# BloodAxe/pytorch-toolbelt

Hardware: AMD Instinct MI355X
Metric: megapixels/sec tiled+d4-TTA merge on 5000x5000 (higher is better)
Workload: dtype f32

## Files before the change

### pytorch_toolbelt_amd/csrc/ptb_channels_last.hip

```cpp
#include "ptb_dispatch.h"
#include "ptb_view_device.h"

namespace ptb {

namespace {

constexpr int CL_THREADS = 256;
constexpr int CL_NC = 4;

template <int IN> struct LdOf { static constexpr int value = IN == PTB_F32 ? 0 : (IN == PTB_F16 ? 2 : 3); };

template <int IN, bool VEC>
__device__ __forceinline__ float4 cl_load(const float* base, long long off, int nc) {
    if constexpr (VEC) {
        return ld4<LdOf<IN>::value>(base, off);
    } else {
        float4 v = make_float4(1.f, 1.f, 1.f, 1.f);
        v.x = widen<IN>(base, off);
        if (nc > 1) v.y = widen<IN>(base, off + 1);
        if (nc > 2) v.z = widen<IN>(base, off + 2);
        if (nc > 3) v.w = widen<IN>(base, off + 3);
        return v;
    }
}

template <int OPK, int IN, bool VEC>
__device__ __forceinline__ float4 cl_reduce_px(const float* __restrict__ base, long long off0, long long view_stride, int nv, int codes, int H, int W,
                                               int C, int i, int j, int c0, int nc, int op, float divisor) {
    float4 v[MAX_VIEWS];
#pragma unroll
    for (int k = 0; k < MAX_VIEWS; ++k) {
        v[k] = make_float4(1.f, 1.f, 1.f, 1.f);
        if (k < nv) {
            const int code = (codes >> (3 * k)) & 7;
            int rr = (code & 1) ? j : i, cc = (code & 1) ? i : j;
            const int rows = (code & 1) ? W : H, cols = (code & 1) ? H : W;
            if (code & 2) rr = rows - 1 - rr;
            if (code & 4) cc = cols - 1 - cc;
            v[k] = cl_load<IN, VEC>(base, off0 + (long long)k * view_stride + ((long long)rr * cols + cc) * C + c0, nc);
        }
    }
    float4 s = make_float4(red_pre<OPK>(v[0].x, op), red_pre<OPK>(v[0].y, op), red_pre<OPK>(v[0].z, op), red_pre<OPK>(v[0].w, op));
#pragma unroll
    for (int k = 1; k < MAX_VIEWS; ++k) {
        if (k < nv) {
            s.x = __fadd_rn(s.x, red_pre<OPK>(v[k].x, op));
            s.y = __fadd_rn(s.y, red_pre<OPK>(v[k].y, op));
            s.z = __fadd_rn(s.z, red_pre<OPK>(v[k].z, op));
            s.w = __fadd_rn(s.w, red_pre<OPK>(v[k].w, op));
        }
    }
    return make_float4(red_post<OPK>(s.x, op, divisor), red_post<OPK>(s.y, op, divisor), red_post<OPK>(s.z, op, divisor),
                       red_post<OPK>(s.w, op, divisor));
}

template <int OPK, int IN, bool VEC>
__device__ __forceinline__ void cl_blend(const ViewArgs& a, const float* __restrict__ base, long long off0, long long view_stride, int li, int lj, int c0,
                                         int nc, float w, float4& acc) {
    const float4 val = round_src4<LdOf<IN>::value>(
        cl_reduce_px<OPK, IN, VEC>(base, off0, view_stride, a.nviews, a.codes, a.H, a.W, a.C, li, lj, c0, nc, a.op, a.divisor), a.round_src);
    acc.x = __fadd_rn(acc.x, __fmul_rn(val.x, w));
    acc.y = __fadd_rn(acc.y, __fmul_rn(val.y, w));
    acc.z = __fadd_rn(acc.z, __fmul_rn(val.z, w));
    acc.w = __fadd_rn(acc.w, __fmul_rn(val.w, w));
}

__device__ __forceinline__ float4 cl_load_planes(const float* p, long long chan_stride, int nc) {
    float4 v = make_float4(0.f, 0.f, 0.f, 0.f);
    v.x = p[0];
    if (nc > 1) v.y = p[chan_stride];
    if (nc > 2) v.z = p[2 * chan_stride];
    if (nc > 3) v.w = p[3 * chan_stride];
    return v;
}
__device__ __forceinline__ void cl_store_planes(float* p, long long chan_stride, int nc, const float4 v) {
    p[0] = v.x;
    if (nc > 1) p[chan_stride] = v.y;
    if (nc > 2) p[2 * chan_stride] = v.z;
    if (nc > 3) p[3 * chan_stride] = v.w;
}
__device__ __forceinline__ float4 cl_div(const float4 s, float n) {
    return make_float4(__fdiv_rn(s.x, n), __fdiv_rn(s.y, n), __fdiv_rn(s.z, n), __fdiv_rn(s.w, n));
}

}

template <int OPK, int IN, bool VEC>
__global__ __launch_bounds__(CL_THREADS) void cl_reduce_kernel(const ViewArgs a, int chrows) {
    const int cpt = a.chunks_x * a.chunks_y;
    const int chunk = blockIdx.x % cpt, t = blockIdx.x / cpt;
    const int cx0 = (chunk % a.chunks_x) * CW, cy0 = (chunk / a.chunks_x) * chrows;
    const int cw = min(CW, a.W - cx0), ch = min(chrows, a.H - cy0);
    const int tx = threadIdx.x & 15, ty = threadIdx.x >> 4;
    const long long off0 = (long long)t * a.src_tile_stride;
    for (int r = ty; r < ch; r += 16) {
        for (int x = tx; x < cw; x += 16) {
            const int i = cy0 + r, j = cx0 + x;
            float* o = a.dst + (long long)t * a.dst_tile_stride + (long long)i * a.dst_row_stride + j;
            for (int c0 = 0; c0 < a.C; c0 += CL_NC) {
                const int nc = min(CL_NC, a.C - c0);
                const float4 val = cl_reduce_px<OPK, IN, VEC>(a.src, off0, a.src_view_stride, a.nviews, a.codes, a.H, a.W, a.C, i, j, c0, nc, a.op, a.divisor);
                cl_store_planes(o + (long long)c0 * a.dst_chan_stride, a.dst_chan_stride, nc, val);
            }
        }
    }
}

template <int OPK, int IN, bool VEC>
__global__ __launch_bounds__(CL_THREADS) void cl_accum_kernel(const ViewArgs a, const CellArgs g, int chrows) {
    const int chunk = blockIdx.x;
    int ci = 0;
    while (ci < a.ncells - 1 && chunk >= g.cells[ci].chunk_end) ++ci;
    const Cell& cell = g.cells[ci];
    const int first = ci ? g.cells[ci - 1].chunk_end : 0;
    const int ncx = (cell.w + CW - 1) / CW;
    const int lc = chunk - first;
    const int cx0 = (lc % ncx) * CW, cy0 = (lc / ncx) * chrows;
    const int cw = min(CW, cell.w - cx0), ch = min(chrows, cell.h - cy0);
    const int ax = cell.ox + cx0, ay = cell.oy + cy0;
    const int nt = cell.ntiles, fresh = cell.fresh, fin = cell.final_;
    const int tx = threadIdx.x & 15, ty = threadIdx.x >> 4;
    for (int r = ty; r < ch; r += 16) {
        for (int x = tx; x < cw; x += 16) {
            const long long pix = (long long)(ay + r) * a.dst_row_stride + ax + x;
            float wv[MAX_COVER];
#pragma unroll
            for (int e = 0; e < MAX_COVER; ++e) {
                wv[e] = 0.f;
                if (e < nt) {
                    const int gt = cell.tile[e];
                    wv[e] = a.weight[(long long)(ay + r - g.tile_y[gt]) * a.W + ax + x - g.tile_x[gt]];
                }
            }
            const float nfull = fin ? a.norm_full[pix] : 1.f;
            if (a.norm != nullptr && !fin) {
                float nacc = fresh ? 0.f : a.norm[pix];
#pragma unroll
                for (int e = 0; e < MAX_COVER; ++e)
                    if (e < nt) nacc = __fadd_rn(nacc, wv[e]);
                a.norm[pix] = nacc;
            }
            for (int c0 = 0; c0 < a.C; c0 += CL_NC) {
                const int nc = min(CL_NC, a.C - c0);
                float* ip = a.dst + (long long)c0 * a.dst_chan_stride + pix;
                float4 acc = fresh ? make_float4(0.f, 0.f, 0.f, 0.f) : cl_load_planes(ip, a.dst_chan_stride, nc);
#pragma unroll
                for (int e = 0; e < MAX_COVER; ++e) {
                    if (e < nt) {
                        const int gt = cell.tile[e];
                        cl_blend<OPK, IN, VEC>(a, a.src, (long long)g.tile_id[gt] * a.src_tile_stride, a.src_view_stride, ay + r - g.tile_y[gt],
                                               ax + x - g.tile_x[gt], c0, nc, wv[e], acc);
                    }
                }
                if (fin) {
                    cl_store_planes(a.merged + (long long)c0 * a.dst_chan_stride + pix, a.dst_chan_stride, nc, cl_div(acc, nfull));
                    if (a.keep_acc) cl_store_planes(ip, a.dst_chan_stride, nc, acc);
                } else {
                    cl_store_planes(ip, a.dst_chan_stride, nc, acc);
                }
            }
        }
    }
}

template <int OPK, int IN, bool VEC>
__global__ __launch_bounds__(CL_THREADS) void cl_band_kernel(const ViewArgs a, const BandArgs g) {
    constexpr int CH = 32;
    const int chunk = blockIdx.x;
    int ci = 0;
    while (ci < a.ncells - 1 && chunk >= g.cells[ci].chunk_end) ++ci;
    const BandCell& cell = g.cells[ci];
    const int first = ci ? g.cells[ci - 1].chunk_end : 0;
    const int ncx = (cell.w + CW - 1) / CW;
    const int lc = chunk - first;
    const int cx0 = (lc % ncx) * CW, cy0 = (lc / ncx) * CH;
    const int cw = min(CW, cell.w - cx0), ch = min(CH, cell.h - cy0);
    const int ax = cell.ox + cx0, ay = cell.oy + cy0;
    const int nt = cell.ntiles;
    const int tx = threadIdx.x & 15, ty = threadIdx.x >> 4;
    for (int r = ty; r < ch; r += 16) {
        for (int x = tx; x < cw; x += 16) {
            const long long pix = (long long)(ay + r) * a.dst_row_stride + ax + x;
            float wv[MAX_COVER];
#pragma unroll
            for (int e = 0; e < MAX_COVER; ++e) {
                wv[e] = 0.f;
                if (e < nt) {
                    const int gt = cell.tile[e];
                    wv[e] = a.weight[(long long)(ay + r - g.tile_y[gt]) * a.W + ax + x - g.tile_x[gt]];
                }
            }
            const float nfull = a.norm_full[pix];
            for (int c0 = 0; c0 < a.C; c0 += CL_NC) {
                const int nc = min(CL_NC, a.C - c0);
                float4 acc = make_float4(0.f, 0.f, 0.f, 0.f);
#pragma unroll
                for (int e = 0; e < MAX_COVER; ++e) {
                    if (e < nt) {
                        const int gt = cell.tile[e];
                        cl_blend<OPK, IN, VEC>(a, static_cast<const float*>(g.tile_src[gt]), 0, g.tile_vs[gt], ay + r - g.tile_y[gt], ax + x - g.tile_x[gt], c0,
                                               nc, wv[e], acc);
                    }
                }
                cl_store_planes(a.merged + (long long)c0 * a.dst_chan_stride + pix, a.dst_chan_stride, nc, cl_div(acc, nfull));
            }
        }
    }
}

template <int OPK, int IN, bool VEC>
__global__ __launch_bounds__(CL_THREADS) void cl_plan_kernel(const ViewArgs a, const BandItem* __restrict__ items, const GroupTiles t) {
    const BandItem* __restrict__ it = items + blockIdx.x;
    const int cwch = it->cwch, partial = it->partial, nt = it->ntiles;
    const int cw = cwch & 0xffff, ch = cwch >> 16;
    const int ax = it->ax, ay = it->ay;
    const int tx = threadIdx.x & 15, ty = threadIdx.x >> 4;
    for (int r = ty; r < ch; r += 16) {
        for (int x = tx; x < cw; x += 16) {
            const long long pix = (long long)(ay + r) * a.dst_row_stride + ax + x;
            float wv[MAX_COVER];
#pragma unroll
            for (int e = 0; e < MAX_COVER; ++e) {
                wv[e] = 0.f;
                if (e < nt) {
                    const unsigned long long cv = it->cover[e];
                    const int lx = (int)((cv >> 16) & 0xffff), ly = (int)((cv >> 32) & 0xffff);
                    wv[e] = a.weight[(long long)(ly + r) * a.W + lx + x];
                }
            }
            float nsum = (a.norm_map && !partial) ? a.norm_full[pix] : 0.f;
#pragma unroll
            for (int e = 0; e < MAX_COVER; ++e)
                if (e < nt && !a.norm_map) nsum = __fadd_rn(nsum, wv[e]);
            for (int c0 = 0; c0 < a.C; c0 += CL_NC) {
                const int nc = min(CL_NC, a.C - c0);
                float4 acc = make_float4(0.f, 0.f, 0.f, 0.f);
#pragma unroll
                for (int e = 0; e < MAX_COVER; ++e) {
                    if (e < nt) {
                        const unsigned long long cv = it->cover[e];
                        const int slot = (int)(cv & 0xffff), lx = (int)((cv >> 16) & 0xffff), ly = (int)((cv >> 32) & 0xffff);
                        cl_blend<OPK, IN, VEC>(a, static_cast<const float*>(t.src[slot]), 0, t.vs[slot], ly + r, lx + x, c0, nc, wv[e], acc);
                    }
                }
                cl_store_planes(a.merged + (long long)c0 * a.dst_chan_stride + pix, a.dst_chan_stride, nc, partial ? acc : cl_div(acc, nsum));
            }
        }
    }
}

template <class F>
static void with_cl_instance(const ViewArgs& a, bool vec, F&& f) {
    with_reduction(a.op, [&](auto opk) { with_src_dtype(a.in_dtype, [&](auto ld) { with_bool(vec, [&](auto v) {
        f(opk, int_c<ld_dtype<ld()>()>{}, v); }); }); });
}

static bool cl_vec_ok(const ViewArgs& a, const void* p, long long stride0, long long stride1) {
    const uintptr_t mask = a.in_dtype == PTB_F32 ? 15u : 7u;
    return a.C % 4 == 0 && (reinterpret_cast<uintptr_t>(p) & mask) == 0 && stride0 % 4 == 0 && stride1 % 4 == 0;
}

void cl_launch_reduce(const ViewArgs& a, int ntiles_out, int ch, hipStream_t s) {
    const dim3 grid((unsigned)ntiles_out * a.chunks_x * a.chunks_y);
    const bool vec = cl_vec_ok(a, a.src, a.src_tile_stride, a.src_view_stride);
    with_cl_instance(a, vec, [&](auto opk, auto in, auto v) {
        hipLaunchKernelGGL((cl_reduce_kernel<opk(), in(), v()>), grid, dim3(CL_THREADS), 0, s, a, ch); });
}

void cl_launch_accum(const ViewArgs& a, const CellArgs& g, int ch, hipStream_t s) {
    const dim3 grid((unsigned)a.total_chunks);
    const bool vec = cl_vec_ok(a, a.src, a.src_tile_stride, a.src_view_stride);
    with_cl_instance(a, vec, [&](auto opk, auto in, auto v) {
        hipLaunchKernelGGL((cl_accum_kernel<opk(), in(), v()>), grid, dim3(CL_THREADS), 0, s, a, g, ch); });
}

void cl_launch_band(const ViewArgs& a, const BandArgs& g, int chunks, hipStream_t s) {
    const dim3 grid((unsigned)chunks);
    bool vec = true;
    for (int ci = 0; ci < a.ncells; ++ci)
        for (int e = 0; e < g.cells[ci].ntiles; ++e) vec = vec && cl_vec_ok(a, g.tile_src[g.cells[ci].tile[e]], g.tile_vs[g.cells[ci].tile[e]], 0);
    with_cl_instance(a, vec, [&](auto opk, auto in, auto v) {
        hipLaunchKernelGGL((cl_band_kernel<opk(), in(), v()>), grid, dim3(CL_THREADS), 0, s, a, g); });
}

void cl_launch_plan(const ViewArgs& a, const BandItem* items, const GroupTiles& t, int n_items, hipStream_t s) {
    const dim3 grid((unsigned)n_items);
    bool vec = true;
    for (int k = 0; k < PLAN_TILES; ++k)
        if (t.src[k]) vec = vec && cl_vec_ok(a, t.src[k], t.vs[k], 0);
    with_cl_instance(a, vec, [&](auto opk, auto in, auto v) {
        hipLaunchKernelGGL((cl_plan_kernel<opk(), in(), v()>), grid, dim3(CL_THREADS), 0, s, a, items, t); });
}

}
```

### pytorch_toolbelt_amd/csrc/ptb_common.h

```cpp
#pragma once
#include <hip/hip_runtime.h>
#include <stdint.h>

#include <type_traits>

#include "../../include/ptb_hip.h"

namespace ptb {

void set_hip_error(hipError_t e);
void set_error_text(const char* text);

inline int check_launch() {
    hipError_t e = hipGetLastError();
    if (e != hipSuccess) {
        set_hip_error(e);
        return PTB_ELAUNCH;
    }
    return PTB_OK;
}

#ifndef PTB_NT_OUT
#define PTB_NT_OUT 1
#endif
__device__ __forceinline__ void out_store4(float* p, const float4 v) {
#if PTB_NT_OUT
    typedef float ptb_v4f __attribute__((ext_vector_type(4)));
    __builtin_nontemporal_store(ptb_v4f{v.x, v.y, v.z, v.w}, reinterpret_cast<ptb_v4f*>(p));
#else
    *reinterpret_cast<float4*>(p) = v;
#endif
}

__device__ __forceinline__ int wave_id() { return __builtin_amdgcn_readfirstlane((int)(threadIdx.x >> 6)); }

inline bool aligned16(const void* p) { return (reinterpret_cast<uintptr_t>(p) & 15u) == 0; }
inline long long up16(long long v) { return (v + 15) & ~15LL; }

inline bool bad_elem_bytes(int eb) { return eb != 1 && eb != 2 && eb != 4 && eb != 8; }
template <int EB>
using label_t = std::conditional_t<EB == 1, unsigned char, std::conditional_t<EB == 2, short, std::conditional_t<EB == 4, int, long long>>>;
inline bool holds(int elem_bytes, long long v) {
    switch (elem_bytes) {
        case 1: return v >= 0 && v <= 255;
        case 2: return v >= -32768 && v <= 32767;
        case 4: return v >= -2147483648LL && v <= 2147483647LL;
        default: return true;
    }
}

constexpr long long MAX_POS = 0x7fffffffLL - 1;
inline int check_shape(int dims, long long B, long long D, long long H, long long W) {
    if ((dims != 2 && dims != 3) || B < 1 || D < 1 || H < 1 || W < 1 || (dims == 2 && D != 1)) return PTB_EINVAL;
    if (D > MAX_POS || H > MAX_POS || W > MAX_POS || H * W > MAX_POS || D * H * W > MAX_POS || B > MAX_POS / (D * H * W)) return PTB_EUNSUPPORTED;
    return PTB_OK;
}

extern int g_chunk_rows;
extern int g_force_scalar;
extern int g_ms_tiled;
extern int g_loss_grid_cap;
extern int g_ms_tile_rows;
extern int g_smf_bwd_stash;
extern int g_ms_strip;
extern int g_band_rows;
extern int g_ms_tile_w;
extern int g_nt_grad_stores;
extern int g_rs_xcd_map;
extern int g_rank_finish_fused;
extern int g_lovasz_fused_dot;
extern int g_stats_pk;
extern int g_band_half_pf;
extern int g_lovasz_rankdot;
extern int g_band_lds_db;
extern int g_band_chan_loop;

}
```

### pytorch_toolbelt_amd/csrc/ptb_core.hip

```cpp
#include <algorithm>
#include <string>

#include "ptb_common.h"

namespace ptb {

static thread_local std::string g_last_error;
int g_chunk_rows = 32;
int g_force_scalar = 0;
int g_band_rows = 64;
int g_ms_tiled = 1;

void set_hip_error(hipError_t e) { g_last_error = hipGetErrorString(e); }
void set_error_text(const char* text) { g_last_error = text ? text : ""; }

template <bool NT>
__global__ __launch_bounds__(256) void merge_div_kernel(const float* __restrict__ image, const float* __restrict__ norm,
                                                        float* __restrict__ out, int C, long long hw4, long long ics4,
                                                        long long ocs4, const float* __restrict__ extra, long long ecs4,
                                                        long long en4) {
    typedef float v4f __attribute__((ext_vector_type(4)));
    const long long stride = (long long)gridDim.x * blockDim.x;
    const v4f* n4 = reinterpret_cast<const v4f*>(norm);
    const v4f* im4 = reinterpret_cast<const v4f*>(image);
    const v4f* ex4 = reinterpret_cast<const v4f*>(extra);
    v4f* o4 = reinterpret_cast<v4f*>(out);
    for (long long i = (long long)blockIdx.x * blockDim.x + threadIdx.x; i < hw4; i += stride) {
        const v4f n = NT ? __builtin_nontemporal_load(&n4[i]) : n4[i];
        for (int c = 0; c < C; ++c) {
            v4f v = NT ? __builtin_nontemporal_load(&im4[c * ics4 + i]) : im4[c * ics4 + i];
            if (i < en4) {
                const v4f e = NT ? __builtin_nontemporal_load(&ex4[c * ecs4 + i]) : ex4[c * ecs4 + i];
                v.x = __fadd_rn(v.x, e.x); v.y = __fadd_rn(v.y, e.y); v.z = __fadd_rn(v.z, e.z); v.w = __fadd_rn(v.w, e.w);
            }
            v4f o;
            o.x = __fdiv_rn(v.x, n.x); o.y = __fdiv_rn(v.y, n.y); o.z = __fdiv_rn(v.z, n.z); o.w = __fdiv_rn(v.w, n.w);
#if PTB_NT_OUT
            __builtin_nontemporal_store(o, &o4[c * ocs4 + i]);
#else
            o4[c * ocs4 + i] = o;
#endif
        }
    }
}

__global__ __launch_bounds__(256) void merge_div_scalar_kernel(const float* __restrict__ image, const float* __restrict__ norm,
                                                               float* __restrict__ out, int C, long long hw, long long ics,
                                                               long long ocs, const float* __restrict__ extra, long long ecs,
                                                               long long en) {
    const long long stride = (long long)gridDim.x * blockDim.x;
    for (long long i = (long long)blockIdx.x * blockDim.x + threadIdx.x; i < hw; i += stride) {
        const float n = norm[i];
        for (int c = 0; c < C; ++c) {
            float v = image[c * ics + i];
            if (i < en) v = __fadd_rn(v, extra[c * ecs + i]);
            out[c * ocs + i] = __fdiv_rn(v, n);
        }
    }
}

__global__ __launch_bounds__(256) void merge_div_masked_kernel(const float* __restrict__ image, const float* __restrict__ norm,
                                                               float* __restrict__ out, int C, int H, int W,
                                                               const uint8_t* __restrict__ mask, int rows) {
    const int nbx = (W + 63) / 64;
    const int bx = blockIdx.x % nbx, by = blockIdx.x / nbx;
    if (!mask[blockIdx.x]) return;
    const long long plane = (long long)H * W;
    const int x0 = bx * 64, y0 = by * rows;
    const int cw = min(64, W - x0), ch = min(rows, H - y0);
    for (int e = threadIdx.x; e < ch * cw; e += blockDim.x) {
        const int r = e / cw, cc = e - r * cw;
        const long long off = (long long)(y0 + r) * W + x0 + cc;
        const float n = norm[off];
        for (int c = 0; c < C; ++c) out[c * plane + off] = __fdiv_rn(image[c * plane + off], n);
    }
}

}

using namespace ptb;

extern "C" int ptb_merge_div_masked(const float* image, const float* norm, float* out, int C, int H, int W, const uint8_t* mask,
                                    int rows, ptb_stream_t stream) {
    if (!image || !norm || !out || !mask || C < 1 || H < 1 || W < 1 || rows < 1) return PTB_EINVAL;
    const long long blocks = (long long)((W + 63) / 64) * ((H + rows - 1) / rows);
    if (blocks > 0x7fffffffLL) return PTB_EUNSUPPORTED;
    hipLaunchKernelGGL(merge_div_masked_kernel, dim3((unsigned)blocks), dim3(256), 0, (hipStream_t)stream, image, norm, out, C, H, W,
                       mask, rows);
    return check_launch();
}

__global__ __launch_bounds__(256) void read_probe_kernel(const float* __restrict__ in, float* __restrict__ sink, long long n4) {
    typedef float v4f __attribute__((ext_vector_type(4)));
    const v4f* p = reinterpret_cast<const v4f*>(in);
    const long long stride = (long long)gridDim.x * blockDim.x;
    float acc = 0.f;
    long long i = (long long)blockIdx.x * blockDim.x + threadIdx.x;
    for (; i + 7 * stride < n4; i += 8 * stride) {
        v4f v[8];
#pragma unroll
        for (int u = 0; u < 8; ++u) v[u] = __builtin_nontemporal_load(&p[i + u * stride]);
#pragma unroll
        for (int u = 0; u < 8; ++u) acc += v[u].x + v[u].y + v[u].z + v[u].w;
    }
    for (; i < n4; i += stride) { const v4f v = __builtin_nontemporal_load(&p[i]); acc += v.x + v.y + v.z + v.w; }
    if (acc == 123.456f) sink[0] = acc;
}

extern "C" int ptb_read_probe(const void* buf, int64_t bytes, float* sink, ptb_stream_t stream) {
    if (!buf || !sink || bytes < 16 || !aligned16(buf)) return PTB_EINVAL;
    hipLaunchKernelGGL(read_probe_kernel, dim3(8192), dim3(256), 0, (hipStream_t)stream, static_cast<const float*>(buf), sink,
                       (long long)(bytes / 16));
    return check_launch();
}

constexpr int PROBE_BUFS = 64;
struct ProbeTable {
    const float* ptr[PROBE_BUFS];
    long long first_chunk[PROBE_BUFS + 1];
};

__global__ __launch_bounds__(256) void read_probe_multi_kernel(const ProbeTable t, int nbufs, float* __restrict__ sink) {
    typedef float v4f __attribute__((ext_vector_type(4)));
    const long long total = t.first_chunk[nbufs];
    float acc = 0.f;
    int b = 0;
    for (long long chunk = blockIdx.x; chunk < total; chunk += gridDim.x) {
        while (chunk >= t.first_chunk[b + 1]) ++b;
        const v4f* p = reinterpret_cast<const v4f*>(t.ptr[b]) + (chunk - t.first_chunk[b]) * 2048 + threadIdx.x;
        v4f v[8];
#pragma unroll
        for (int u = 0; u < 8; ++u) v[u] = __builtin_nontemporal_load(&p[u * 256]);
#pragma unroll
        for (int u = 0; u < 8; ++u) acc += v[u].x + v[u].y + v[u].z + v[u].w;
    }
    if (acc == 123.456f) sink[0] = acc;
}

extern "C" int64_t ptb_read_probe_multi(const void* const* bufs, const int64_t* bytes, int n, float* sink, int workgroups, ptb_stream_t stream) {
    if (!bufs || !bytes || !sink || n < 1 || n > PROBE_BUFS) return PTB_EINVAL;
    ProbeTable t{};
    long long chunks = 0;
    for (int i = 0; i < n; ++i) {
        if (!bufs[i] || bytes[i] < 0 || !aligned16(bufs[i])) return PTB_EINVAL;
        t.ptr[i] = static_cast<const float*>(bufs[i]);
        t.first_chunk[i] = chunks;
        chunks += bytes[i] / 32768;
    }
    t.first_chunk[n] = chunks;
    if (!chunks) return PTB_EINVAL;
    const int grid = (int)std::min<long long>(chunks, workgroups > 0 ? workgroups : 8192);
    hipLaunchKernelGGL(read_probe_multi_kernel, dim3(grid), dim3(256), 0, (hipStream_t)stream, t, n, sink);
    const int rc = check_launch();
    return rc != PTB_OK ? rc : (int64_t)chunks * 32768;
}

__global__ __launch_bounds__(256) void sums_finalize_kernel(const double* __restrict__ slots, int nslots, int n, double* __restrict__ out,
                                                            const int* __restrict__ flag) {
    const bool bad = flag && *flag;
    for (int i = threadIdx.x; i < n; i += blockDim.x) {
        double t = 0.0;
        for (int s = 0; s < nslots; ++s) t += slots[(long long)s * n + i];
        out[i] = bad ? (double)__builtin_nanf("") : t;
    }
}

extern "C" int ptb_sums_finalize(const double* slot_sums, int nslots, int n, double* out, const int* error_flag, ptb_stream_t stream) {
    if (!slot_sums || !out || nslots < 1 || n < 1) return PTB_EINVAL;
    hipLaunchKernelGGL(sums_finalize_kernel, dim3(1), dim3(256), 0, (hipStream_t)stream, slot_sums, nslots, n, out, error_flag);
    return check_launch();
}

extern "C" int ptb_version(void) { return 102; }

extern "C" const char* ptb_last_hip_error(void) { return g_last_error.c_str(); }

namespace {
enum Check {
    BOOL,
    BIT0,
    RANGE,
    CLAMP,
    SET,
};
struct Tunable { int key; int* var; Check check; int v[3]; };
const Tunable kTunables[] = {
    {0, &g_chunk_rows, SET, {16, 32, 64}},
    {1, &g_force_scalar, BOOL, {}},
    {3, &g_ms_tiled, BOOL, {}},
    {4, &g_loss_grid_cap, RANGE, {0, 0x7fffffff}},
    {6, &g_ms_tile_rows, SET, {16, 32, 64}},
    {7, &g_smf_bwd_stash, SET, {0, 2, 4}},
    {9, &g_ms_strip, RANGE, {0, 64}},
    {11, &g_band_rows, SET, {32, 64, 64}},
    {15, &g_ms_tile_w, SET, {64, 128, 128}},
    {16, &g_nt_grad_stores, BOOL, {}},
    {17, &g_rs_xcd_map, BIT0, {}},
    {18, &g_rank_finish_fused, BOOL, {}},
    {19, &g_lovasz_fused_dot, BOOL, {}},
    {20, &g_stats_pk, BOOL, {}},
    {21, &g_band_half_pf, CLAMP, {0, 2}},
    {23, &g_lovasz_rankdot, BOOL, {}},
    {25, &g_band_lds_db, BOOL, {}},
    {27, &g_band_chan_loop, BOOL, {}},
};
}

extern "C" int ptb_set_tunable(int key, int value) {
    for (const Tunable& t : kTunables) {
        if (t.key != key) continue;
        switch (t.check) {
            case BOOL: value = value ? 1 : 0; break;
            case BIT0: value &= 1; break;
            case RANGE: if (value < t.v[0] || value > t.v[1]) return PTB_EINVAL; break;
            case CLAMP: value = std::min(std::max(value, t.v[0]), t.v[1]); break;
            case SET: if (value != t.v[0] && value != t.v[1] && value != t.v[2]) return PTB_EINVAL; break;
        }
        *t.var = value;
        return PTB_OK;
    }
    return PTB_EINVAL;
}

extern "C" int ptb_merge_div_ex(const float* image, const float* norm, float* out, int C, int64_t HW, int64_t image_cs,
                                int64_t out_cs, const float* extra, int64_t extra_cs, int64_t extra_n, ptb_stream_t stream) {
    if (!image || !norm || !out || C < 1 || HW < 0 || image_cs < HW || out_cs < HW) return PTB_EINVAL;
    if (extra_n < 0 || extra_n > HW || (extra_n > 0 && (!extra || extra_cs < extra_n))) return PTB_EINVAL;
    if (HW == 0) return PTB_OK;
    hipStream_t s = (hipStream_t)stream;
    const bool vec = !g_force_scalar && HW % 4 == 0 && image_cs % 4 == 0 && out_cs % 4 == 0 && aligned16(image) &&
                     aligned16(norm) && aligned16(out) &&
                     (extra_n == 0 || (extra_n % 4 == 0 && extra_cs % 4 == 0 && aligned16(extra)));
    if (vec) {
        const long long hw4 = HW / 4;
        const long long want = (hw4 + 255) / 256;
        const int blocks = (int)(want < 256 * 16 ? want : 256 * 16);
        hipLaunchKernelGGL(merge_div_kernel<false>, dim3(blocks), dim3(256), 0, s, image, norm, out, C, hw4, (long long)image_cs / 4,
                                (long long)out_cs / 4, extra, (long long)extra_cs / 4, (long long)extra_n / 4);
    } else {
        const long long want = (HW + 255) / 256;
        const int blocks = (int)(want < 256 * 16 ? want : 256 * 16);
        hipLaunchKernelGGL(merge_div_scalar_kernel, dim3(blocks), dim3(256), 0, s, image, norm, out, C, (long long)HW,
                           (long long)image_cs, (long long)out_cs, extra, (long long)extra_cs, (long long)extra_n);
    }
    return check_launch();
}

template <int VEC>
__global__ __launch_bounds__(256) void rect_add_kernel(float* __restrict__ dst, const float* __restrict__ src, int C, int rows, int cols,
                                                       long long dst_cs, long long dst_rs) {
    typedef float v4f __attribute__((ext_vector_type(4)));
    const int x = (blockIdx.x * 256 + threadIdx.x) * VEC;
    if (x >= cols) return;
    for (long long cr = blockIdx.y; cr < (long long)C * rows; cr += gridDim.y) {
        const int c = (int)(cr / rows), r = (int)(cr - (long long)c * rows);
        float* d = dst + c * dst_cs + r * dst_rs + x;
        const float* s = src + cr * cols + x;
        if (VEC == 4) {
            const v4f b = __builtin_nontemporal_load(reinterpret_cast<const v4f*>(s));
            *reinterpret_cast<v4f*>(d) = *reinterpret_cast<v4f*>(d) + b;
        } else {
            *d += *s;
        }
    }
}

extern "C" int ptb_rect_add(float* dst, const float* src, int C, int rows, int cols, int64_t dst_cs, int64_t dst_rs,
                            ptb_stream_t stream) {
    if (!dst || !src || C < 1 || rows < 0 || cols < 0 || dst_rs < cols || dst_cs < (int64_t)rows * dst_rs) return PTB_EINVAL;
    if (rows == 0 || cols == 0) return PTB_OK;
    const long long cr = (long long)C * rows;
    const int gy = (int)(cr < 65535 ? cr : 65535);
    hipStream_t s = (hipStream_t)stream;
    const bool vec = !g_force_scalar && cols % 4 == 0 && dst_cs % 4 == 0 && dst_rs % 4 == 0 && aligned16(dst) && aligned16(src);
    if (vec)
        hipLaunchKernelGGL(rect_add_kernel<4>, dim3((cols / 4 + 255) / 256, gy), dim3(256), 0, s, dst, src, C, rows, cols,
                           (long long)dst_cs, (long long)dst_rs);
    else
        hipLaunchKernelGGL(rect_add_kernel<1>, dim3((cols + 255) / 256, gy), dim3(256), 0, s, dst, src, C, rows, cols,
                           (long long)dst_cs, (long long)dst_rs);
    return check_launch();
}

extern "C" int ptb_merge_div(const float* image, const float* norm, float* out, int C, int64_t HW, ptb_stream_t stream) {
    return ptb_merge_div_ex(image, norm, out, C, HW, HW, HW, nullptr, 0, 0, stream);
}
```

### pytorch_toolbelt_amd/csrc/ptb_view_device.h

```cpp
#pragma once
#include <initializer_list>

#include "ptb_common.h"
#include "ptb_dispatch.h"

namespace ptb {

constexpr int MAX_VIEWS = 8;
constexpr int MAX_T = 4;
constexpr int MAX_CELLS = 64;
constexpr int MAX_COVER = 4;
constexpr int MAX_GROUP = 64;
constexpr int CW = 64;

constexpr int lds_tiles(int nv, int codes) {
    if (codes < 0) return nv < MAX_T ? nv : MAX_T;
    int n = 0;
    for (int k = 0; k < nv; ++k) n += (codes >> (3 * k)) & 1;
    return n;
}

struct Cell {
    int ox, oy, w, h;
    int chunk_end;
    int ntiles;
    int fresh;
    int final_;
    int tile[MAX_COVER];
};

struct CellArgs {
    Cell cells[MAX_CELLS];
    int tile_x[MAX_GROUP];
    int tile_y[MAX_GROUP];
    int tile_id[MAX_GROUP];
};

struct ViewArgs {
    const float* src;
    float* dst;
    float* norm;
    const float* weight;
    float* merged;
    const float* norm_full;
    int H, W, C;
    long long src_view_stride;
    long long src_tile_stride;
    long long dst_tile_stride;
    long long dst_chan_stride;
    int dst_row_stride;
    int nviews;
    int codes;
    int tiles_per_view;
    int src_tile_mod;
    int op;
    float divisor;
    float scale;
    int chunks_x, chunks_y;
    int ncells, total_chunks;
    int in_dtype;
    int keep_acc;
    int round_src;
    int chan_loop;
    int lds_db;
    int norm_map;
};

enum { MODE_REDUCE = 0, MODE_PERVIEW = 1, MODE_ACCUM = 2 };

constexpr float kEps = 1e-6f;
constexpr float kOneMinusEps = (float)(1.0 - 1e-6);

__device__ __forceinline__ float fast_exp(float x) { return __builtin_amdgcn_exp2f(x * 1.4426950408889634f); }
__device__ __forceinline__ float fast_log(float x) { return __builtin_amdgcn_logf(x) * 0.6931471805599453f; }
__device__ __forceinline__ float fast_rcp(float x) { return __builtin_amdgcn_rcpf(x); }

template <int OPK>
__device__ __forceinline__ float red_pre(float x, int op) {
    if (OPK == 0) return x;
    switch (op) {
        case PTB_RED_GMEAN: return fast_log(x);
        case PTB_RED_HMEAN: return fast_rcp(x < kEps ? kEps : x);
        case PTB_RED_HARMONIC1P: return fast_rcp(x + 1.0f);
        case PTB_RED_LOGODD: {
            float p = x < kEps ? kEps : (x > kOneMinusEps ? kOneMinusEps : x);
            return fast_log(p * fast_rcp(1.0f - p));
        }
        case PTB_RED_LOG1P: return fast_log(1.0f + x);
        default: return x;
    }
}

__device__ __forceinline__ float div_views(float s, float divisor) {
    const unsigned bits = __float_as_uint(divisor);
    if ((bits & 0x807FFFFFu) == 0 && bits != 0) return s * __uint_as_float(0x7F000000u - bits);
    return s / divisor;
}

template <int OPK>
__device__ __forceinline__ float red_post(float s, int op, float divisor) {
    if (OPK == 0) return divisor == 1.0f ? s : div_views(s, divisor);
    const float m = div_views(s, divisor);
    switch (op) {
        case PTB_RED_GMEAN: return fast_exp(m);
        case PTB_RED_HMEAN: return fast_rcp(m < kEps ? kEps : m);
        case PTB_RED_HARMONIC1P: return fast_rcp(m) - 1.0f;
        case PTB_RED_LOGODD: { const float e = fast_exp(m); return e * fast_rcp(1.0f + e); }
        case PTB_RED_LOG1P: return fast_exp(m) - 1.0f;
        default: return m;
    }
}

__device__ __forceinline__ float red_dpost(float out, int op) {
    switch (op) {
        case PTB_RED_GMEAN: return out;
        case PTB_RED_HMEAN: return out >= 1.0f / kEps ? 0.f : -out * out;
        case PTB_RED_HARMONIC1P: return -(out + 1.0f) * (out + 1.0f);
        case PTB_RED_LOGODD: return out * (1.0f - out);
        case PTB_RED_LOG1P: return out + 1.0f;
        default: return 1.0f;
    }
}
__device__ __forceinline__ float red_dpre(float x, int op) {
    switch (op) {
        case PTB_RED_GMEAN: return 1.0f / x;
        case PTB_RED_HMEAN: return x < kEps ? 0.f : -1.0f / (x * x);
        case PTB_RED_HARMONIC1P: return -1.0f / ((x + 1.0f) * (x + 1.0f));
        case PTB_RED_LOGODD: return (x < kEps || x > kOneMinusEps) ? 0.f : 1.0f / (x * (1.0f - x));
        case PTB_RED_LOG1P: return 1.0f / (1.0f + x);
        default: return 1.0f;
    }
}

__device__ __forceinline__ int swz(int i, int j) { return i * CW + ((((j >> 2) ^ (i >> 2)) & 15) << 2) + (j & 3); }

__device__ __forceinline__ int swzg(int i, int j) {
    return i * CW + ((((j >> 2) ^ (i >> 2)) & 15) << 2) + ((j & 3) ^ ((i >> 4) & 2));
}
__device__ __forceinline__ float4 unswz4(const float4 t, int i) {
    return (i & 32) ? make_float4(t.z, t.w, t.x, t.y) : t;
}

typedef float v4f __attribute__((ext_vector_type(4)));

template <bool NT>
__device__ __forceinline__ float4 ld16(const float* p) {
    const v4f* q = reinterpret_cast<const v4f*>(p);
    const v4f v = NT ? __builtin_nontemporal_load(q) : *q;
    return make_float4(v.x, v.y, v.z, v.w);
}

template <int LD>
__device__ __forceinline__ float4 ld4(const float* base, long long off) {
    if constexpr (LD <= 1) {
        return ld16<LD == 1>(base + off);
    } else if constexpr (LD == 2) {
        typedef _Float16 h4 __attribute__((ext_vector_type(4)));
        const h4 v = __builtin_nontemporal_load(reinterpret_cast<const h4*>(reinterpret_cast<const _Float16*>(base) + off));
        return make_float4((float)v.x, (float)v.y, (float)v.z, (float)v.w);
    } else {
        typedef unsigned short u4 __attribute__((ext_vector_type(4)));
        const u4 v = __builtin_nontemporal_load(reinterpret_cast<const u4*>(reinterpret_cast<const unsigned short*>(base) + off));
        return make_float4(__uint_as_float((unsigned)v.x << 16), __uint_as_float((unsigned)v.y << 16),
                           __uint_as_float((unsigned)v.z << 16), __uint_as_float((unsigned)v.w << 16));
    }
}

typedef unsigned int raw2 __attribute__((ext_vector_type(2)));
template <int LD> struct RawOf { typedef raw2 type; };
template <> struct RawOf<0> { typedef v4f type; };
template <> struct RawOf<1> { typedef v4f type; };
template <int LD>
__device__ __forceinline__ typename RawOf<LD>::type ld4_raw(const float* base, long long off) {
    if constexpr (LD <= 1) {
        const v4f* q = reinterpret_cast<const v4f*>(base + off);
        return LD == 1 ? __builtin_nontemporal_load(q) : *q;
    } else {
        return __builtin_nontemporal_load(reinterpret_cast<const raw2*>(reinterpret_cast<const unsigned short*>(base) + off));
    }
}
template <int LD>
__device__ __forceinline__ float4 widen4(const typename RawOf<LD>::type r) {
    if constexpr (LD <= 1) {
        return make_float4(r.x, r.y, r.z, r.w);
    } else if constexpr (LD == 2) {
        const unsigned lo = r.x, hi = r.y;
        return make_float4((float)__builtin_bit_cast(_Float16, (unsigned short)(lo & 0xffffu)), (float)__builtin_bit_cast(_Float16, (unsigned short)(lo >> 16)),
                           (float)__builtin_bit_cast(_Float16, (unsigned short)(hi & 0xffffu)), (float)__builtin_bit_cast(_Float16, (unsigned short)(hi >> 16)));
    } else {
        return make_float4(__uint_as_float(r.x << 16), __uint_as_float(r.x & 0xFFFF0000u), __uint_as_float(r.y << 16), __uint_as_float(r.y & 0xFFFF0000u));
    }
}

template <int LD>
__device__ __forceinline__ float round_src1(float x) {
    if constexpr (LD == 2) {
        return (float)(_Float16)x;
    } else if constexpr (LD == 3) {
        return (float)(__bf16)x;
    } else {
        return x;
    }
}
template <int LD>
__device__ __forceinline__ float4 round_src4(const float4 v, int on) {
    if constexpr (LD <= 1) return v;
    else return on ? make_float4(round_src1<LD>(v.x), round_src1<LD>(v.y), round_src1<LD>(v.z), round_src1<LD>(v.w)) : v;
}

__device__ __forceinline__ float comp(const float4& v, int m) { return m == 0 ? v.x : (m == 1 ? v.y : (m == 2 ? v.z : v.w)); }

template <int OUT>
__device__ __forceinline__ unsigned short half_bits(float f) {
    if constexpr (OUT == PTB_F16) return __builtin_bit_cast(unsigned short, (_Float16)f);
    else return __builtin_bit_cast(unsigned short, (__bf16)f);
}

template <int IN>
__device__ __forceinline__ float widen(const void* p, long long i) {
    if constexpr (IN == PTB_F32) return static_cast<const float*>(p)[i];
    else if constexpr (IN == PTB_F16) return (float)static_cast<const _Float16*>(p)[i];
    else if constexpr (IN == PTB_BF16) return __uint_as_float((unsigned)static_cast<const unsigned short*>(p)[i] << 16);
    else if constexpr (IN == PTB_U8) return (float)static_cast<const uint8_t*>(p)[i];
    else if constexpr (IN == PTB_I16) return (float)static_cast<const int16_t*>(p)[i];
    else return (float)static_cast<const uint16_t*>(p)[i];
}

template <int LD>
constexpr int ld_dtype() { return LD == 2 ? PTB_F16 : (LD == 3 ? PTB_BF16 : PTB_F32); }

template <int OUT>
__device__ __forceinline__ void out_store4_as(float* dst, long long off, const float4 v) {
    if constexpr (OUT == PTB_F32) {
        out_store4(dst + off, v);
    } else {
        typedef unsigned int u2 __attribute__((ext_vector_type(2)));
        const u2 w{(unsigned)half_bits<OUT>(v.x) | ((unsigned)half_bits<OUT>(v.y) << 16), (unsigned)half_bits<OUT>(v.z) | ((unsigned)half_bits<OUT>(v.w) << 16)};
        u2* p = reinterpret_cast<u2*>(reinterpret_cast<unsigned short*>(dst) + off);
#if PTB_NT_OUT
        __builtin_nontemporal_store(w, p);
#else
        *p = w;
#endif
    }
}

template <int CH, bool NONLIN, int OUT = PTB_F32>
__device__ __forceinline__ void scatter_chunk(const ViewArgs& a, int B, int b, int c, int x0, int y0, int cw, int ch, float4 v,
                                              float* st, int tid) {
    constexpr int SL = CH / 4;
    const int q = tid & 15, r = tid >> 4;
    const bool act = r < ch && 4 * q < cw;
    const long long plane = (long long)a.H * a.W;
    bool any_t = false;
    for (int k = 0; k < a.nviews; ++k) {
        const int code = (a.codes >> (3 * k)) & 7;
        if (code & 1) { any_t = true; continue; }
        if (act) {
            const int i = (code & 2) ? a.H - 1 - (y0 + r) : y0 + r;
            const int j = (code & 4) ? a.W - 4 - (x0 + 4 * q) : x0 + 4 * q;
            const long long off = (((long long)k * B + b) * a.C + c) * plane + (long long)i * a.W + j;
            float4 w = (code & 4) ? make_float4(v.w, v.z, v.y, v.x) : v;
            if (NONLIN) {
                const float4 x4 = ld16<true>(a.weight + off);
                w.x *= red_dpre(x4.x, a.op); w.y *= red_dpre(x4.y, a.op); w.z *= red_dpre(x4.z, a.op); w.w *= red_dpre(x4.w, a.op);
            }
            out_store4_as<OUT>(a.dst, off, w);
        }
    }
    if (!any_t) return;
    if (act) {
#pragma unroll
        for (int m = 0; m < 4; ++m) {
            const int col = 4 * q + m;
            st[col * CH + ((((r >> 2) ^ (col >> 2)) & (SL - 1)) << 2) + (r & 3)] = comp(v, m);
        }
    }
    __syncthreads();
    const int ii = tid / SL, qq = tid % SL;
    if (ii < cw && 4 * qq < ch) {
        const float4 t = *reinterpret_cast<const float4*>(&st[ii * CH + (((qq ^ (ii >> 2)) & (SL - 1)) << 2)]);
        for (int k = 0; k < a.nviews; ++k) {
            const int code = (a.codes >> (3 * k)) & 7;
            if (!(code & 1)) continue;
            const int i = (code & 4) ? a.W - 1 - (x0 + ii) : x0 + ii;
            const int j = (code & 2) ? a.H - 4 - (y0 + 4 * qq) : y0 + 4 * qq;
            const long long off = (((long long)k * B + b) * a.C + c) * plane + (long long)i * a.W + j;
            float4 w = (code & 2) ? make_float4(t.w, t.z, t.y, t.x) : t;
            if (NONLIN) {
                const float4 x4 = ld16<true>(a.weight + off);
                w.x *= red_dpre(x4.x, a.op); w.y *= red_dpre(x4.y, a.op); w.z *= red_dpre(x4.z, a.op); w.w *= red_dpre(x4.w, a.op);
            }
            out_store4_as<OUT>(a.dst, off, w);
        }
    }
}

constexpr int pack_codes(std::initializer_list<int> l) {
    int v = 0, k = 0;
    for (int c : l) v |= c << (3 * k++);
    return v;
}
constexpr int CODES_ID = 0;
constexpr int CODES_FLIPLR = pack_codes({0, 4});
constexpr int CODES_FLIPUD = pack_codes({0, 2});
constexpr int CODES_FLIPS = pack_codes({0, 4, 2});
constexpr int CODES_D2 = pack_codes({0, 4, 2, 6});
constexpr int CODES_D4 = pack_codes({0, 5, 6, 3, 1, 4, 7, 2});

template <class F>
void with_view_set(int nviews, int codes, F&& f) {
    if (nviews == 1 && codes == CODES_ID) f(int_c<1>{}, int_c<CODES_ID>{});
    else if (nviews == 2 && codes == CODES_FLIPLR) f(int_c<2>{}, int_c<CODES_FLIPLR>{});
    else if (nviews == 2 && codes == CODES_FLIPUD) f(int_c<2>{}, int_c<CODES_FLIPUD>{});
    else if (nviews == 3 && codes == CODES_FLIPS) f(int_c<3>{}, int_c<CODES_FLIPS>{});
    else if (nviews == 4 && codes == CODES_D2) f(int_c<4>{}, int_c<CODES_D2>{});
    else if (nviews == 8 && codes == CODES_D4) f(int_c<8>{}, int_c<CODES_D4>{});
    else f(int_c<8>{}, int_c<-1>{});
}


template <int CH, int NV, int CODES, int OPK>
__device__ __forceinline__ float4 gather_tail(float4 (&v)[NV], int nv_rt, int codes_rt, int cw, int ch, int op, float divisor, float* lds, int tid,
                                              bool more_entries) {
    constexpr int QPR = CH / 4;
    const int q = tid & 15, r = tid >> 4;
    const int rr = tid / QPR, qq = tid % QPR;
    const bool act = (r < ch) && (4 * q < cw);
    const bool tact = (rr < cw) && (4 * qq < ch);
    const int nv = CODES >= 0 ? NV : nv_rt;
    const int codes = CODES >= 0 ? CODES : codes_rt;
    int tb = 0;
#pragma unroll
    for (int k = 0; k < NV; ++k) {
        if (k < nv && ((codes >> (3 * k)) & 1)) {
            const int code = (codes >> (3 * k)) & 7;
            float* buf = lds + tb * (CW * CH);
            ++tb;
            if (tact) {
                const int jl = (code & 2) ? cw - 1 - rr : rr;
#pragma unroll
                for (int m = 0; m < 4; ++m) {
                    const int cc = 4 * qq + m;
                    const int il = (code & 4) ? ch - 1 - cc : cc;
                    if constexpr (CH == 64 && CODES >= 0) buf[swzg(il, jl)] = comp(v[k], m);
                    else buf[swz(il, jl)] = comp(v[k], m);
                }
            }
        }
    }
    if (tb) {
        __syncthreads();
        tb = 0;
#pragma unroll
        for (int k = 0; k < NV; ++k) {
            if (k < nv && ((codes >> (3 * k)) & 1)) {
                const float* buf = lds + tb * (CW * CH);
                ++tb;
                v[k] = act ? *reinterpret_cast<const float4*>(buf + swz(r, 4 * q)) : make_float4(1.f, 1.f, 1.f, 1.f);
                if constexpr (CH == 64 && CODES >= 0) v[k] = unswz4(v[k], r);
            }
        }
        if (more_entries) __syncthreads();
    }

    float4 s = make_float4(red_pre<OPK>(v[0].x, op), red_pre<OPK>(v[0].y, op), red_pre<OPK>(v[0].z, op), red_pre<OPK>(v[0].w, op));
#pragma unroll
    for (int k = 1; k < NV; ++k) {
        if (k < nv) {
            s.x = __fadd_rn(s.x, red_pre<OPK>(v[k].x, op));
            s.y = __fadd_rn(s.y, red_pre<OPK>(v[k].y, op));
            s.z = __fadd_rn(s.z, red_pre<OPK>(v[k].z, op));
            s.w = __fadd_rn(s.w, red_pre<OPK>(v[k].w, op));
        }
    }
    return make_float4(red_post<OPK>(s.x, op, divisor), red_post<OPK>(s.y, op, divisor), red_post<OPK>(s.z, op, divisor),
                       red_post<OPK>(s.w, op, divisor));
}


template <int CH, int NV, int CODES, int OPK, int LD>
__device__ __forceinline__ float4 gather_reduce(const float* __restrict__ src, long long plane, long long view_stride, int nv_rt,
                                                int codes_rt, int H, int W, int lx, int ly, int cw, int ch, int op,
                                                float divisor, float* lds, int tid, bool more_entries) {
    constexpr int QPR = CH / 4;
    const int q = tid & 15, r = tid >> 4;
    const int rr = tid / QPR, qq = tid % QPR;
    const bool act = (r < ch) && (4 * q < cw);
    const bool tact = (rr < cw) && (4 * qq < ch);
    const int nv = CODES >= 0 ? NV : nv_rt;
    const int codes = CODES >= 0 ? CODES : codes_rt;

    float4 v[NV];
#pragma unroll
    for (int k = 0; k < NV; ++k) {
        v[k] = make_float4(1.f, 1.f, 1.f, 1.f);
        if (k < nv) {
            const int code = (codes >> (3 * k)) & 7;
            const long long p = plane + (long long)k * view_stride;
            if (!(code & 1)) {
                if (act) {
                    const int i = ly + r, j = lx + 4 * q;
                    const int row = (code & 2) ? H - 1 - i : i;
                    const int col = (code & 4) ? W - 4 - j : j;
                    const float4 t = ld4<LD>(src, p + (long long)row * W + col);
                    v[k] = (code & 4) ? make_float4(t.w, t.z, t.y, t.x) : t;
                }
            } else if (tact) {
                const int R0 = (code & 2) ? H - lx - cw : lx;
                const int C0 = (code & 4) ? W - ly - ch : ly;
                v[k] = ld4<LD>(src, p + (long long)(R0 + rr) * W + C0 + 4 * qq);
            }
        }
    }

    return gather_tail<CH, NV, CODES, OPK>(v, nv_rt, codes_rt, cw, ch, op, divisor, lds, tid, more_entries);
}

template <int CH, int NV, int CODES, int LD>
__device__ __forceinline__ void gather_load_raw(const float* __restrict__ src, long long plane, long long view_stride, int nv_rt, int codes_rt, int H,
                                                int W, int lx, int ly, int cw, int ch, int tid, typename RawOf<LD>::type (&raw)[NV]) {
    constexpr int QPR = CH / 4;
    const int q = tid & 15, r = tid >> 4;
    const int rr = tid / QPR, qq = tid % QPR;
    const bool act = (r < ch) && (4 * q < cw);
    const bool tact = (rr < cw) && (4 * qq < ch);
    const int nv = CODES >= 0 ? NV : nv_rt;
    const int codes = CODES >= 0 ? CODES : codes_rt;
#pragma unroll
    for (int k = 0; k < NV; ++k) {
        raw[k] = typename RawOf<LD>::type{};
        if (k < nv) {
            const int code = (codes >> (3 * k)) & 7;
            const long long p = plane + (long long)k * view_stride;
            if (!(code & 1)) {
                if (act) {
                    const int i = ly + r, j = lx + 4 * q;
                    const int row = (code & 2) ? H - 1 - i : i;
                    const int col = (code & 4) ? W - 4 - j : j;
                    raw[k] = ld4_raw<LD>(src, p + (long long)row * W + col);
                }
            } else if (tact) {
                const int R0 = (code & 2) ? H - lx - cw : lx;
                const int C0 = (code & 4) ? W - ly - ch : ly;
                raw[k] = ld4_raw<LD>(src, p + (long long)(R0 + rr) * W + C0 + 4 * qq);
            }
        }
    }
}
template <int CH, int NV, int CODES, int LD>
__device__ __forceinline__ void gather_widen(const typename RawOf<LD>::type (&raw)[NV], int nv_rt, int codes_rt, int cw, int ch, int tid, float4 (&v)[NV]) {
    constexpr int QPR = CH / 4;
    const int q = tid & 15, r = tid >> 4;
    const int rr = tid / QPR, qq = tid % QPR;
    const bool act = (r < ch) && (4 * q < cw);
    const bool tact = (rr < cw) && (4 * qq < ch);
    const int nv = CODES >= 0 ? NV : nv_rt;
    const int codes = CODES >= 0 ? CODES : codes_rt;
#pragma unroll
    for (int k = 0; k < NV; ++k) {
        v[k] = make_float4(1.f, 1.f, 1.f, 1.f);
        if (k < nv) {
            const int code = (codes >> (3 * k)) & 7;
            if (!(code & 1)) {
                if (act) {
                    const float4 t = widen4<LD>(raw[k]);
                    v[k] = (code & 4) ? make_float4(t.w, t.z, t.y, t.x) : t;
                }
            } else if (tact) {
                v[k] = widen4<LD>(raw[k]);
            }
        }
    }
}

constexpr int BAND_CELLS = 40, BAND_TILES = 48;
struct BandCell {
    int ox, oy, w, h;
    int chunk_end;
    int ntiles;
    int tile[MAX_COVER];
};
struct BandArgs {
    BandCell cells[BAND_CELLS];
    int tile_x[BAND_TILES], tile_y[BAND_TILES];
    const void* tile_src[BAND_TILES];
    long long tile_vs[BAND_TILES];
};

constexpr int PLAN_TILES = 224;
constexpr int PLAN_CH = 32;

struct BandItem {
    int ax, ay;
    int cwch;
    int ntiles;
    int partial;
    int pad[3];
    unsigned long long cover[MAX_COVER];
};
static_assert(sizeof(BandItem) == 64, "BandItem layout");

struct GroupTiles {
    const void* src[PLAN_TILES];
    long long vs[PLAN_TILES];
};

void cl_launch_reduce(const ViewArgs& a, int ntiles_out, int ch, hipStream_t s);
void cl_launch_accum(const ViewArgs& a, const CellArgs& g, int ch, hipStream_t s);
void cl_launch_band(const ViewArgs& a, const BandArgs& g, int chunks, hipStream_t s);
void cl_launch_plan(const ViewArgs& a, const BandItem* items, const GroupTiles& t, int n_items, hipStream_t s);

struct ActCfg { int activation; float temperature; };
bool ta_view_set_ok(int nviews, int codes);
void ta_launch_accum(const ViewArgs& a, const CellArgs& g, int ch, bool src_cl, int activation, float temperature, hipStream_t s);
void ta_launch_plan(const ViewArgs& a, const BandItem* items, const GroupTiles& t, int n_items, bool src_cl, int activation, float temperature,
                    hipStream_t s);

}
```

Baseline: 12200.

## Add vectorized channels-last plan kernel with DPP quad transpose and load prefetch

Adds a new channels-last plan kernel that loads four channels per thread as one vector, fuses the D4 view reduction and weighted tile merge, and software-pipelines the next step's loads. Results are transposed across lane quads with DPP moves so each lane writes a contiguous float4 in channel-first output. It replaces the generic plan kernel when channels divide by four, no norm map is used and offsets fit in 32 bits. The risks are extra register pressure from the prefetch buffers and specialization only for known view-code sets.

```diff
diff --git a/pytorch_toolbelt_amd/csrc/ptb_channels_last.hip b/pytorch_toolbelt_amd/csrc/ptb_channels_last.hip
--- a/pytorch_toolbelt_amd/csrc/ptb_channels_last.hip
+++ b/pytorch_toolbelt_amd/csrc/ptb_channels_last.hip
@@ -288,6 +288,7 @@
     bool vec = true;
     for (int k = 0; k < PLAN_TILES; ++k)
         if (t.src[k]) vec = vec && cl_vec_ok(a, t.src[k], t.vs[k], 0);
+    if (cl_vec_plan_launch(a, vec, items, t, n_items, s)) return;
     with_cl_instance(a, vec, [&](auto opk, auto in, auto v) {
         hipLaunchKernelGGL((cl_plan_kernel<opk(), in(), v()>), grid, dim3(CL_THREADS), 0, s, a, items, t); });
 }
diff --git a/pytorch_toolbelt_amd/csrc/ptb_channels_last_plan.hip b/pytorch_toolbelt_amd/csrc/ptb_channels_last_plan.hip
--- /dev/null
+++ b/pytorch_toolbelt_amd/csrc/ptb_channels_last_plan.hip
@@ -0,0 +1,162 @@
+#include "ptb_dispatch.h"
+#include "ptb_view_device.h"
+
+namespace ptb {
+
+int g_cl_vec_plan = 1;
+
+namespace {
+
+constexpr int CLP_THREADS = 256;
+
+__device__ __forceinline__ float quad_xor1(float v) { return __int_as_float(__builtin_amdgcn_mov_dpp(__float_as_int(v), 0xB1, 0xf, 0xf, true)); }
+__device__ __forceinline__ float quad_xor2(float v) { return __int_as_float(__builtin_amdgcn_mov_dpp(__float_as_int(v), 0x4E, 0xf, 0xf, true)); }
+
+__device__ __forceinline__ float4 quad_transpose(float4 v, int l) {
+    const bool o1 = (l & 1) != 0, o2 = (l & 2) != 0;
+    float r0 = quad_xor1(o1 ? v.x : v.y), r1 = quad_xor1(o1 ? v.z : v.w);
+    if (o1) { v.x = r0; v.z = r1; } else { v.y = r0; v.w = r1; }
+    r0 = quad_xor2(o2 ? v.x : v.z); r1 = quad_xor2(o2 ? v.y : v.w);
+    if (o2) { v.x = r0; v.y = r1; } else { v.z = r0; v.w = r1; }
+    return v;
+}
+
+template <int LD>
+__device__ __forceinline__ typename RawOf<LD>::type ld_raw_at(const char* base, unsigned off) {
+    typedef typename RawOf<LD>::type Raw;
+    const Raw* q = reinterpret_cast<const Raw*>(base + off);
+    if constexpr (LD == 0) return *q;
+    else return __builtin_nontemporal_load(q);
+}
+
+struct Step { int eg, cg, bx, by; };
+
+}
+
+template <int NV, int CODES, int OPK, int LD>
+__global__ __launch_bounds__(CLP_THREADS) void cl_vec_group_kernel(const ViewArgs a, const BandItem* __restrict__ items, const GroupTiles t) {
+    constexpr int EPS = NV <= 2 ? MAX_COVER : 1;
+    typedef typename RawOf<LD>::type Raw;
+    const BandItem* __restrict__ it = items + blockIdx.x;
+    const int cwch = it->cwch, partial = it->partial, nt = it->ntiles;
+    const int cw = cwch & 0xffff, ch = cwch >> 16;
+    constexpr bool FP = LD >= 2 && lds_tiles(NV, CODES) > 0;
+    const int lane = threadIdx.x & 63, wv = threadIdx.x >> 6;
+    const int tx = FP ? ((wv & 1) << 3) | (lane & 7) : threadIdx.x & 15, ty = FP ? ((wv >> 1) << 3) | (lane >> 3) : threadIdx.x >> 4;
+    const int nbx = (cw + 15) >> 4, ncg = a.C >> 2;
+    const int neg = nt > EPS ? (nt + EPS - 1) / EPS : 1;
+    const int nsteps = neg * ncg * nbx * ((ch + 15) >> 4);
+
+    auto advance = [&](Step& s) {
+        if (++s.eg < neg) return;
+        s.eg = 0;
+        if (++s.cg < ncg) return;
+        s.cg = 0;
+        if (++s.bx < nbx) return;
+        s.bx = 0;
+        ++s.by;
+    };
+    const unsigned px_b = (unsigned)a.C * (unsigned)sizeof(Raw) / 4u;
+    const unsigned row_b = px_b * (unsigned)a.W;
+    auto request = [&](const Step& s, Raw (&raw)[EPS][NV], float (&w)[EPS]) {
+        const int x = s.bx * 16 + tx, r = s.by * 16 + ty;
+        const bool g = x < cw && r < ch;
+#pragma unroll
+        for (int q = 0; q < EPS; ++q) {
+            const int e = s.eg * EPS + q;
+            if (e < nt && g) {
+                const unsigned long long cv = it->cover[e];
+                const int slot = (int)(cv & 0xffff), lx = (int)((cv >> 16) & 0xffff), ly = (int)((cv >> 32) & 0xffff);
+                const int i = ly + r, j = lx + x;
+                w[q] = a.weight[(long long)i * a.W + j];
+                const char* base = static_cast<const char*>(t.src[slot]) + (size_t)s.cg * sizeof(Raw);
+                const long long vs_b = t.vs[slot] * (long long)(sizeof(Raw) / 4);
+                const unsigned i_px = (unsigned)i * px_b, j_px = (unsigned)j * px_b, i_row = (unsigned)i * row_b, j_row = (unsigned)j * row_b;
+#pragma unroll
+                for (int k = 0; k < NV; ++k) {
+                    const int code = (CODES >> (3 * k)) & 7;
+                    const unsigned rr_b = (code & 1) ? j_row : i_row, cc_b = (code & 1) ? i_px : j_px;
+                    const unsigned rows = (code & 1) ? a.W : a.H, cols = (code & 1) ? a.H : a.W;
+                    const unsigned mirror = ((code & 2) ? (rows - 1) * row_b : 0u) + ((code & 4) ? (cols - 1) * px_b : 0u);
+                    const unsigned off = mirror + ((code & 2) ? 0u - rr_b : rr_b) + ((code & 4) ? 0u - cc_b : cc_b);
+                    const char* vb = base + (long long)k * vs_b;
+                    raw[q][k] = ld_raw_at<LD>(vb, off);
+                }
+            }
+        }
+    };
+
+    Raw nxt[EPS][NV] = {};
+    float wn[EPS] = {};
+    Step sn{0, 0, 0, 0};
+    request(sn, nxt, wn);
+    float4 acc = make_float4(0.f, 0.f, 0.f, 0.f);
+    float nsum = 0.f;
+    for (int s = 0; s < nsteps; ++s) {
+        const Step sc = sn;
+        Raw cur[EPS][NV];
+        float wc[EPS];
+#pragma unroll
+        for (int q = 0; q < EPS; ++q) {
+            wc[q] = wn[q];
+#pragma unroll
+            for (int k = 0; k < NV; ++k) cur[q][k] = nxt[q][k];
+        }
+        advance(sn);
+        if (s + 1 < nsteps) request(sn, nxt, wn);
+        if (sc.eg == 0) {
+            acc = make_float4(0.f, 0.f, 0.f, 0.f);
+            nsum = 0.f;
+        }
+#pragma unroll
+        for (int q = 0; q < EPS; ++q) {
+            if (sc.eg * EPS + q < nt) {
+                const float4 v0 = widen4<LD>(cur[q][0]);
+                float4 sum = make_float4(red_pre<OPK>(v0.x, a.op), red_pre<OPK>(v0.y, a.op), red_pre<OPK>(v0.z, a.op), red_pre<OPK>(v0.w, a.op));
+#pragma unroll
+                for (int k = 1; k < NV; ++k) {
+                    const float4 v = widen4<LD>(cur[q][k]);
+                    sum.x = __fadd_rn(sum.x, red_pre<OPK>(v.x, a.op));
+                    sum.y = __fadd_rn(sum.y, red_pre<OPK>(v.y, a.op));
+                    sum.z = __fadd_rn(sum.z, red_pre<OPK>(v.z, a.op));
+                    sum.w = __fadd_rn(sum.w, red_pre<OPK>(v.w, a.op));
+                }
+                const float4 val = round_src4<LD>(make_float4(red_post<OPK>(sum.x, a.op, a.divisor), red_post<OPK>(sum.y, a.op, a.divisor),
+                                                              red_post<OPK>(sum.z, a.op, a.divisor), red_post<OPK>(sum.w, a.op, a.divisor)), a.round_src);
+                acc.x = __fadd_rn(acc.x, __fmul_rn(val.x, wc[q]));
+                acc.y = __fadd_rn(acc.y, __fmul_rn(val.y, wc[q]));
+                acc.z = __fadd_rn(acc.z, __fmul_rn(val.z, wc[q]));
+                acc.w = __fadd_rn(acc.w, __fmul_rn(val.w, wc[q]));
+                nsum = __fadd_rn(nsum, wc[q]);
+            }
+        }
+        if (sc.eg == neg - 1) {
+            float4 o = acc;
+            if (!partial) o = make_float4(__fdiv_rn(acc.x, nsum), __fdiv_rn(acc.y, nsum), __fdiv_rn(acc.z, nsum), __fdiv_rn(acc.w, nsum));
+            const int l = tx & 3;
+            o = quad_transpose(o, l);
+            const int x = sc.bx * 16 + tx, r = sc.by * 16 + ty;
+            if (x < cw && r < ch) {
+                float* p = a.merged + (long long)(4 * sc.cg + l) * a.dst_chan_stride + (long long)(it->ay + r) * a.dst_row_stride + it->ax + (x - l);
+                *reinterpret_cast<float4*>(p) = o;
+            }
+        }
+    }
+}
+
+bool cl_vec_plan_launch(const ViewArgs& a, bool vec, const BandItem* items, const GroupTiles& t, int n_items, hipStream_t s) {
+    if (!g_cl_vec_plan || !vec || a.C % 4 != 0 || a.norm_map != 0) return false;
+    if ((long long)a.H * a.W * a.C * (a.in_dtype == PTB_F32 ? 4 : 2) >= (1LL << 31)) return false;
+    bool launched = false;
+    with_view_set(a.nviews, a.codes, [&](auto nv, auto codes) {
+        if constexpr (codes() >= 0) {
+            with_src_dtype(a.in_dtype, [&](auto ld) { with_reduction(a.op, [&](auto opk) {
+                hipLaunchKernelGGL((cl_vec_group_kernel<nv(), codes(), opk(), (ld() == 1 ? 0 : ld())>), dim3((unsigned)n_items), dim3(CLP_THREADS), 0, s, a,
+                                   items, t); }); });
+            launched = true;
+        }
+    });
+    return launched;
+}
+
+}
diff --git a/pytorch_toolbelt_amd/csrc/ptb_common.h b/pytorch_toolbelt_amd/csrc/ptb_common.h
--- a/pytorch_toolbelt_amd/csrc/ptb_common.h
+++ b/pytorch_toolbelt_amd/csrc/ptb_common.h
@@ -74,5 +74,6 @@
 extern int g_lovasz_rankdot;
 extern int g_band_lds_db;
 extern int g_band_chan_loop;
+extern int g_cl_vec_plan;
 
 }
diff --git a/pytorch_toolbelt_amd/csrc/ptb_core.hip b/pytorch_toolbelt_amd/csrc/ptb_core.hip
--- a/pytorch_toolbelt_amd/csrc/ptb_core.hip
+++ b/pytorch_toolbelt_amd/csrc/ptb_core.hip
@@ -203,6 +203,7 @@
     {23, &g_lovasz_rankdot, BOOL, {}},
     {25, &g_band_lds_db, BOOL, {}},
     {27, &g_band_chan_loop, BOOL, {}},
+    {28, &g_cl_vec_plan, BOOL, {}},
 };
 }
 
diff --git a/pytorch_toolbelt_amd/csrc/ptb_view_device.h b/pytorch_toolbelt_amd/csrc/ptb_view_device.h
--- a/pytorch_toolbelt_amd/csrc/ptb_view_device.h
+++ b/pytorch_toolbelt_amd/csrc/ptb_view_device.h
@@ -511,6 +511,8 @@
 void cl_launch_band(const ViewArgs& a, const BandArgs& g, int chunks, hipStream_t s);
 void cl_launch_plan(const ViewArgs& a, const BandItem* items, const GroupTiles& t, int n_items, hipStream_t s);
 
+bool cl_vec_plan_launch(const ViewArgs& a, bool vec, const BandItem* items, const GroupTiles& t, int n_items, hipStream_t s);
+
 struct ActCfg { int activation; float temperature; };
 bool ta_view_set_ok(int nviews, int codes);
 void ta_launch_accum(const ViewArgs& a, const CellArgs& g, int ch, bool src_cl, int activation, float temperature, hipStream_t s);
```

Measured after the change: 12200 (median of 2 runs). No clear change (+0.0%).
